# refresh-bio/kmer-db

Measured on AMD Instinct MI355X. Metric: all2all k-mer pair-comparisons/sec, higher is better.
Workload: dtype u32

## Files before the change

### kmer-db_amd/csrc/a2a_blocks.hip

```cpp
#include "device_common.h"
#include "engine_internal.h"

#include "prim.h"

#include <algorithm>
#include <chrono>
#include <cmath>
#include <cstdio>
#include <cstdlib>
#include <cstring>

enum : uint32_t {
    KCTR_CHUNKS = 0,
    KCTR_POOL_OVERFLOW,
    KCTR_PAIR_OVERFLOW,
    KCTR_NWIDE,
    KCTR_LIST_OVERFLOW,
    KCTR_RAW = 5,
    KCTR_RECORDS = 6,
    KCTR_RECORDS_HI = 7,
    KCTR_SLOW = 8,
    KCTR_WIDE_OVERFLOW = 9,
    KCTR_WIDE_RECORDS = 10,
    KCTR_ROWJOBS = 11,
// ... 815 lines not shown
                    n_direct += (uint32_t)__popcll(__ballot(mine));
                    if (!(q.dbg & 2u)) {
                    const TrConst trc = tr_const(lane);
                    const unsigned long long Rt = transpose64(mine ? F0 : 0ull, trc);
                    unsigned long long ra0, ra1;
                    {
                        const auto a = __builtin_amdgcn_permlane32_swap((uint32_t)Rt, (uint32_t)Rt, false, false);
                        const auto b = __builtin_amdgcn_permlane32_swap((uint32_t)(Rt >> 32), (uint32_t)(Rt >> 32), false, false);
                        ra0 = ((unsigned long long)b[0] << 32) | a[0];
                        ra1 = ((unsigned long long)b[1] << 32) | a[1];
                    }
                    wbuf[wave][lane] = (unsigned char)(mine ? w : 0u);
                    lds_sync();
                    const uint32_t half = lane >> 5;
                    auto spread = [&](unsigned long long word, uint32_t shift, const unsigned long long* lut) -> k2_v4i {
                        const uint32_t f = (uint32_t)(word >> shift) & 0xFFFFu;
                        k2_v4i r;
                        const unsigned long long lo = lut[f & 0xFFu], hi = lut[f >> 8];
                        r[0] = (int)(uint32_t)lo; r[1] = (int)(uint32_t)(lo >> 32); r[2] = (int)(uint32_t)hi; r[3] = (int)(uint32_t)(hi >> 32);
                        return r;
                    };
    #pragma unroll 1
                    for (uint32_t kh = 0; kh < 2; ++kh) {
                        const uint32_t shift = 32u * kh + 16u * half;
                        k2_v4i a0 = spread(ra0, shift, lut_ff), a1 = spread(ra1, shift, lut_ff);
                        const k2_v4i b0 = spread(ra0, shift, lut_01), b1 = spread(ra1, shift, lut_01);
                        const k2_v4i wv = *(const k2_v4i*)(wbuf[wave] + shift);
                        a0 &= wv; a1 &= wv;
                        c00 = __builtin_amdgcn_mfma_i32_32x32x32_i8(a0, b0, c00, 0, 0, 0);
                        c10 = __builtin_amdgcn_mfma_i32_32x32x32_i8(a1, b0, c10, 0, 0, 0);
                        c11 = __builtin_amdgcn_mfma_i32_32x32x32_i8(a1, b1, c11, 0, 0, 0);
                    }
                    lds_sync();
                    }
                    d0 = d0 && !mine;
                }
            }
            if (MODE == 0 && !q.all_wide) {
                unsigned long long pend = __ballot(d0);
                while (pend) {
                    const uint32_t X0 = bcast(w0, (uint32_t)__builtin_ctzll(pend));
                    const bool mine = d0 && w0 == X0;
                    const unsigned long long bc = __ballot(mine);
                    const Resv r = arena_reserve(A, q.pool, X0, tri32(X0) + X0, (uint32_t)__popcll(bc), lane);
                    if (mine) rec_store_diag(q.pool, resv_slot(r, (uint32_t)__popcll(bc & lt_mask)), F0, w);
                    pend &= ~bc;
                }
            } else {
                rec_emit<ROWS>(A, pv, RT, d0, w0, F0, F0, w, tri32(w0) + w0, lane, lt_mask);
            }
        };
        if (!DIRECT) first_block_records();
        {
            const bool act2 = act && F1 != 0;
            if (__ballot(act2)) {
                rec_emit<ROWS>(A, pv, RT, act2, w1, F1, F0, w, tri32(w1) + w0, lane, lt_mask);
                rec_emit<ROWS>(A, pv, RT, act2 && __popcll(F1) >= 2, w1, F1, F1, w, tri32(w1) + w1, lane, lt_mask);
            }
        }
        if (base + WAVE < end) {
            uint32_t m = dep;
#pragma unroll
            for (int s = 1; s < WAVE; s <<= 1) {
                const uint32_t o = (uint32_t)__shfl_down((int)m, s, WAVE);
                if (lane + (uint32_t)s < (uint32_t)WAVE) m = o < m ? o : m;
            }
            uint32_t later = (uint32_t)__shfl_down((int)m, 1, WAVE);
            if (lane == (uint32_t)WAVE - 1u) later = 0xFFFFFFFFu;
            if (valid && dep < later) { chain_m[dep - 1u] = make_ulonglong2(S.m0, S.m1); chain_b[dep - 1u] = S.bw; }
            lds_sync();
        }
        if (DIRECT) first_block_records();
    }
    if (DIRECT && curX != BNONE && !(q.dbg & 1u)) dflush();
    KARG(NParams) qe = kernarg_reread<NParams>();
    if (DIRECT && lane == 0 && n_direct) atomicAdd(&qe->direct_ctr[(seg % KMDB_SUBPOOLS) * 16u], n_direct);
    if (FLAT && lane == 0) { qe->slice_cnt[seg] = flat_n; if (flat_n) atomicAdd(&qe->direct_ctr[(seg % KMDB_SUBPOOLS) * 16u], flat_n); }
    if (lane == 0) qe->wide_slice_cnt[seg] = n_flagged;
    if constexpr (MODE == 0) arena_finish(A, q.pool, lane);
    if constexpr (ROWS) rowtab_finish(RT, pv, lane);
    else arena_finish_wide(A, pv, lane);
}

constexpr uint32_t K2D_SLICES = 2;
struct DParams {
    const unsigned long long* dmask;
    const uint32_t* dwx;
    const uint32_t* slice_cnt;
    uint32_t n_segs, nseg_nodes, slices;
    uint32_t* M;
    uint32_t N, bwidth;
    unsigned char* touched;
};
__global__ __launch_bounds__(256) __attribute__((amdgpu_waves_per_eu(4, 8))) void k2d_kernel(const DParams q) {
    __shared__ unsigned long long lut_ff[256], lut_01[256];
    __shared__ __attribute__((aligned(16))) unsigned char wbuf[4][64];
    {
        unsigned long long v = 0;
#pragma unroll
        for (int i = 0; i < 8; ++i) v |= ((threadIdx.x >> i) & 1u) ? 0xFFull << (8 * i) : 0ull;
        lut_ff[threadIdx.x] = v;
        lut_01[threadIdx.x] = v & 0x0101010101010101ull;
        __syncthreads();
    }
    const uint32_t lane = threadIdx.x & 63u, wave = threadIdx.x >> 6;
    const uint32_t half = lane >> 5, l31 = lane & 31u;
    const uint32_t s0 = (blockIdx.x * 4u + wave) * q.slices;
    if (s0 >= q.n_segs) return;
    const uint32_t s1 = s0 + q.slices < q.n_segs ? s0 + q.slices : q.n_segs;
    const TrConst trc = tr_const(lane);
    auto spread = [&](unsigned long long word, uint32_t shift, const unsigned long long* lut) -> k2_v4i {
        const uint32_t f = (uint32_t)(word >> shift) & 0xFFFFu;
        k2_v4i r;
        const unsigned long long lo = lut[f & 0xFFu], hi = lut[f >> 8];
        r[0] = (int)(uint32_t)lo; r[1] = (int)(uint32_t)(lo >> 32); r[2] = (int)(uint32_t)hi; r[3] = (int)(uint32_t)(hi >> 32);
        return r;
    };
    uint32_t s = s0, n = q.slice_cnt[s0], b = 0;
    auto skip_empty = [&]() { while (b >= n && s + 1u < s1) { ++s; n = q.slice_cnt[s]; b = 0; } };
    skip_empty();
    unsigned long long nm = 0; uint32_t nwx = 0;
    auto fetch = [&]() {
        nm = 0; nwx = 0;
        if (b + lane < n) { const size_t i = (size_t)s * q.nseg_nodes + b + lane; nm = q.dmask[i]; nwx = q.dwx[i]; }
    };
    if (b < n) fetch();
    unsigned long long m = 0, pend = 0;
    uint32_t wx = 0;
    auto next_step = [&]() -> bool {
        if (b >= n) return false;
        m = nm; wx = nwx;
        b += WAVE;
        skip_empty();
        if (b < n) fetch();
        pend = __ballot(m != 0ull);
        return true;
    };
    for (;;) {
        while (!pend && next_step()) {}
        if (!pend) break;
        const uint32_t X0 = bcast(wx >> 8, (uint32_t)__builtin_ctzll(pend));
        k2_v16i c00 = {}, c10 = {}, c11 = {};
        for (;;) {
            const bool mine = ((pend >> lane) & 1ull) && (wx >> 8) == X0;
            const unsigned long long bm = __ballot(mine);
            if (!bm) break;
            pend &= ~bm;
            const unsigned long long Rt = transpose64(mine ? m : 0ull, trc);
            unsigned long long ra0, ra1;
            {
                const auto a = __builtin_amdgcn_permlane32_swap((uint32_t)Rt, (uint32_t)Rt, false, false);
                const auto c = __builtin_amdgcn_permlane32_swap((uint32_t)(Rt >> 32), (uint32_t)(Rt >> 32), false, false);
                ra0 = ((unsigned long long)c[0] << 32) | a[0];
                ra1 = ((unsigned long long)c[1] << 32) | a[1];
            }
            wbuf[wave][lane] = (unsigned char)(mine ? (wx & 0xFFu) : 0u);
            lds_sync();
#pragma unroll 1
            for (uint32_t kh = 0; kh < 2; ++kh) {
                const uint32_t shift = 32u * kh + 16u * half;
                k2_v4i a0 = spread(ra0, shift, lut_ff), a1 = spread(ra1, shift, lut_ff);
                const k2_v4i b0 = spread(ra0, shift, lut_01), b1 = spread(ra1, shift, lut_01);
                const k2_v4i wv = *(const k2_v4i*)(wbuf[wave] + shift);
                a0 &= wv; a1 &= wv;
                c00 = __builtin_amdgcn_mfma_i32_32x32x32_i8(a0, b0, c00, 0, 0, 0);
                c10 = __builtin_amdgcn_mfma_i32_32x32x32_i8(a1, b0, c10, 0, 0, 0);
                c11 = __builtin_amdgcn_mfma_i32_32x32x32_i8(a1, b1, c11, 0, 0, 0);
            }
            lds_sync();
            if (pend || !next_step()) break;
        }
        const uint32_t rb = X0 * q.bwidth;
        uint32_t* const Mb = q.M + (tri64((uint64_t)rb) + rb);
        const uint32_t lim = q.N - rb;
        uint32_t h4 = 4u * half, lc = l31;
        asm volatile("" : "+v"(h4), "+v"(lc));
#pragma unroll
        for (int r = 0; r < 16; ++r) {
            const uint32_t row0 = (uint32_t)((r & 3) + 8 * (r >> 2)) + h4, row1 = row0 + 32u;
            const uint32_t o0 = rb * row0 + row0 * (row0 - 1u) / 2u + lc, o1 = rb * row1 + row1 * (row1 - 1u) / 2u + lc;
            const uint32_t v00 = (uint32_t)c00[r], v10 = (uint32_t)c10[r], v11 = (uint32_t)c11[r];
            if (v00 && lc < row0 && row0 < lim) atomicAdd(Mb + o0, v00);
            if (v10 && row1 < lim) atomicAdd(Mb + o1, v10);
            if (v11 && lc < row0 && row1 < lim) atomicAdd(Mb + o1 + 32u, v11);
        }
        if (lane == 0 && q.touched) q.touched[tri32(X0) + X0] = 1;
    }
}

constexpr uint32_t WSL_THREADS = 1024;
__global__ __launch_bounds__(WSL_THREADS) void wide_slices_kernel(const uint32_t* __restrict__ slice_cnt, uint32_t n_segs, uint32_t* __restrict__ slice_base,
                                                                   uint32_t* __restrict__ wide_base, uint32_t n_words, uint32_t* __restrict__ counters) {
    __shared__ uint32_t wtot[WSL_THREADS / WAVE];
    const uint32_t lane = threadIdx.x & 63u, wave = threadIdx.x >> 6;
    constexpr uint32_t NW = WSL_THREADS / WAVE;
    const uint32_t share = ((n_segs + NW - 1u) / NW + 63u) & ~63u;
    const uint32_t lo = wave * share < n_segs ? wave * share : n_segs;
    const uint32_t hi = n_segs - lo < share ? n_segs : lo + share;
    constexpr uint32_t U = 8;
    uint32_t sum = 0;
    for (uint32_t i0 = lo; i0 < hi; i0 += U * WAVE) {
        uint32_t v[U];
#pragma unroll
        for (uint32_t j = 0; j < U; ++j) { const uint32_t i = i0 + j * WAVE + lane; v[j] = i < hi ? slice_cnt[i] : 0u; }
#pragma unroll
        for (uint32_t j = 0; j < U; ++j) sum += v[j];
    }
#pragma unroll
    for (int d = 32; d >= 1; d >>= 1) sum += (uint32_t)__shfl_xor((int)sum, d, WAVE);
    if (lane == 0) wtot[wave] = sum;
    __syncthreads();
    uint32_t run = 0, total = 0;
    for (uint32_t k = 0; k < NW; ++k) { const uint32_t t = wtot[k]; if (k < wave) run += t; total += t; }
    for (uint32_t i0 = lo; i0 < hi; i0 += U * WAVE) {
        uint32_t v[U];
#pragma unroll
        for (uint32_t j = 0; j < U; ++j) { const uint32_t i = i0 + j * WAVE + lane; v[j] = i < hi ? slice_cnt[i] : 0u; }
#pragma unroll
        for (uint32_t j = 0; j < U; ++j) {
            const uint32_t i = i0 + j * WAVE + lane;
            const uint32_t incl = wave_incl_scan(v[j], lane);
            if (i < hi) slice_base[i] = run + incl - v[j];
            run += bcast(incl, WAVE - 1u);
        }
    }
    if (threadIdx.x == 0) { slice_base[n_segs] = total; wide_base[n_words] = total; counters[KCTR_NWIDE] = total; }
}
__global__ __launch_bounds__(256) void wide_expand_kernel(const unsigned long long* __restrict__ bits, uint32_t* __restrict__ base, const uint32_t* __restrict__ slice_base,
                                                          uint32_t words_per_slice, uint32_t slice_shift, uint32_t n_words, uint32_t* __restrict__ widx, uint32_t cap) {
    const uint32_t i = blockIdx.x * blockDim.x + threadIdx.x;
    unsigned long long b = 0;
    uint32_t o = 0;
    if (i < n_words) {
        b = bits[i];
        o = slice_base[slice_shift != 0xFFFFFFFFu ? i >> slice_shift : i / words_per_slice] + base[i];
        base[i] = o;
    }
    while (b) {
        const uint32_t k = (uint32_t)__builtin_ctzll(b);
        b &= b - 1;
        if (o < cap) widx[o] = i * 64u + k;
        ++o;
    }
}

constexpr uint32_t BLK_NONE = 0xFFFFu;
struct LSum { unsigned long long lm; uint32_t c, fb, lb; };
__device__ __forceinline__ LSum lsum_none() { return LSum{0ull, 0u, BLK_NONE, BLK_NONE}; }
__device__ __forceinline__ LSum lsum_merge(const LSum& A, const LSum& B) {
    if (B.c == 0u) return A;
    if (A.c == 0u) return B;
    const bool seam = A.lb == B.fb;
    return LSum{(B.c == 1u && seam) ? (A.lm | B.lm) : B.lm, A.c + B.c - (seam ? 1u : 0u), A.fb, B.lb};
}
__device__ __forceinline__ LSum lsum_shfl(const LSum& s, int src) {
    return LSum{shfl64(s.lm, src), (uint32_t)__shfl((int)s.c, src, WAVE), (uint32_t)__shfl((int)s.fb, src, WAVE), (uint32_t)__shfl((int)s.lb, src, WAVE)};
}
__device__ __forceinline__ LSum lsum_shfl_up(const LSum& s, int d) {
    return LSum{shfl_up64(s.lm, d), (uint32_t)__shfl_up((int)s.c, d, WAVE), (uint32_t)__shfl_up((int)s.fb, d, WAVE), (uint32_t)__shfl_up((int)s.lb, d, WAVE)};
}
__device__ __forceinline__ LSum lsum_of_fn(uint32_t fb, const ulonglong2& fm) {
    const uint32_t b0 = fb & 0xFFFFu, b1 = fb >> 16;
    if (b0 == BLK_NONE) return lsum_none();
    if (b1 == BLK_NONE) return LSum{fm.x, 1u, b0, b0};
    return LSum{fm.y, 2u, b0, b1};
}

struct L2View {
    uint32_t on, min_blocks;
    uint32_t node_cap, W;
// ... 1335 lines not shown
    const uint32_t t = blockIdx.x * blockDim.x + threadIdx.x;
    const uint64_t i0 = (uint64_t)t * q.stride + (t * 2654435761u) % q.stride;
    const uint32_t node = (uint32_t)i0;
    const bool on = i0 < q.P && q.w[node] != 0 && q.nl[node] >= 2u;
    uint32_t nblk[EST_NW], lower_first[EST_NW];
#pragma unroll
    for (int c = 0; c < EST_NW; ++c) { nblk[c] = 0; lower_first[c] = 0xFFFFFFFFu; }
    int32_t y = on ? (int32_t)node : -1;
    while (y >= 0) {
        const uint2 km = q.k0in[y];
        const uint32_t l = kmdb_k0_l(km), last = kmdb_k0_last(km);
        if (l) {
            const uint64_t pos = q.blkbase[(uint32_t)y >> 8] + q.bitrel[y];
            uint32_t sum = 0;
            if (l > 1) { BitCursor c(q.bits, pos); for (uint32_t k = 0; k + 1 < l; ++k) sum += c.next(); }
            uint32_t id = last - sum;
            uint32_t fb[EST_NW], cb[EST_NW];
#pragma unroll
            for (int c = 0; c < EST_NW; ++c) { fb[c] = __umulhi(id, q.magics[c]); cb[c] = fb[c]; nblk[c] += 1; }
            if (l > 1) {
                BitCursor c2(q.bits, pos);
                for (uint32_t k = 0; k + 1 < l; ++k) {
                    id += c2.next();
#pragma unroll
                    for (int c = 0; c < EST_NW; ++c) { const uint32_t b = __umulhi(id, q.magics[c]); nblk[c] += b != cb[c]; cb[c] = b; }
                }
            }
#pragma unroll
            for (int c = 0; c < EST_NW; ++c) { nblk[c] -= cb[c] == lower_first[c]; lower_first[c] = fb[c]; }
        }
        y = q.parent[y];
    }
    const uint32_t lane = threadIdx.x & 63u;
#pragma unroll
    for (int c = 0; c < EST_NW; ++c) {
        const unsigned long long recs = (unsigned long long)nblk[c] * (nblk[c] + 1u) / 2u;
        unsigned long long rn = on && nblk[c] >= 1u && nblk[c] <= 2u ? 1ull : 0ull;
        unsigned long long rg = on ? recs - rn : 0ull;
        unsigned long long r2 = on && nblk[c] >= q.l2_min ? recs : 0ull;
#pragma unroll
        for (int d = 32; d >= 1; d >>= 1) { rn += shfl64(rn, (int)(lane ^ (uint32_t)d)); rg += shfl64(rg, (int)(lane ^ (uint32_t)d)); r2 += shfl64(r2, (int)(lane ^ (uint32_t)d)); }
        if (lane == 0) { if (rn) atomicAdd(&q.out[c], rn); if (rg) atomicAdd(&q.out[EST_NW + c], rg); if (r2) atomicAdd(&q.out[2 * EST_NW + 1 + c], r2); }
    }
    const unsigned long long nb = __ballot(on);
    if (lane == 0 && nb) atomicAdd(&q.out[2 * EST_NW], (unsigned long long)__popcll(nb));
}

__global__ void pair_estimate_kernel(const uint2* __restrict__ k0in, const uint32_t* __restrict__ bitrel, const uint64_t* __restrict__ blkbase,
                                     const uint64_t* __restrict__ bits, uint32_t P, uint32_t stride, BlockMap bm, unsigned long long* __restrict__ out) {
    const uint32_t t = blockIdx.x * blockDim.x + threadIdx.x;
    const uint64_t i0 = (uint64_t)t * stride + (t * 2654435761u) % stride;
    unsigned long long need = 0;
    if (i0 < P) {
        const uint2 km = k0in[i0];
        const uint32_t l = kmdb_k0_l(km), last = kmdb_k0_last(km);
        if (l > 1) {
            BitCursor c(bits, blkbase[(uint32_t)i0 >> 8] + bitrel[i0]);
            uint32_t span = 0;
            for (uint32_t k = 0; k + 1 < l; ++k) span += c.next();
            const uint32_t nb = bm.blk(last) - bm.blk(last - span);
            need = nb < l - 1u ? nb : l - 1u;
        }
    }
    const uint32_t lane = threadIdx.x & 63u;
#pragma unroll
    for (int d = 32; d >= 1; d >>= 1) need += shfl64(need, (int)(lane ^ (uint32_t)d));
    if (lane == 0 && need) atomicAdd(out, need);
}

inline uint32_t wide_digit_bits(int key_bits) { return (uint32_t)(32 - key_bits - 2); }

constexpr uint32_t K1W_RUN_NODES = 256;
struct BlocksKnobs {
    uint32_t block_width = 0;
    bool dense_narrow = false;
    int k1n_mode = 2;
    int k1n_minw = 3;
    int row_mode = -1;
    bool rec_packed = true;
    bool l2 = true;
    uint32_t l2_min = L2_MIN_BLOCKS;
    uint64_t slices = 0;
    uint64_t pool_percent = 0;
    uint32_t k2d_slices = K2D_SLICES;
    bool k2d_early = true;
    uint32_t k1w_run = K1W_RUN_NODES;
    uint32_t k1w_waves = 0;
};
BlocksKnobs blocks_read_knobs() {
    BlocksKnobs k;
    auto env = [](const char* name) -> const char* { const char* e = getenv(name); return e && *e ? e : nullptr; };
    if (const char* e = env("KMDB_BLOCK_WIDTH")) { const uint32_t w = (uint32_t)strtoul(e, nullptr, 10); if (w >= 32 && w <= 64) k.block_width = w; }
    if (const char* e = env("KMDB_DENSE")) k.dense_narrow = atoi(e) >= 2;
    if (const char* e = env("KMDB_K1N_MODE")) k.k1n_mode = std::max(0, std::min(2, atoi(e)));
    if (const char* e = env("KMDB_K1N_MINW")) k.k1n_minw = atoi(e);
    if (const char* e = env("KMDB_ROW_MODE")) k.row_mode = atoi(e) != 0;
    if (const char* e = env("KMDB_REC_PACKED")) k.rec_packed = e[0] != '0';
    if (const char* e = env("KMDB_L2")) k.l2 = e[0] != '0';
    if (const char* e = env("KMDB_L2_MIN")) k.l2_min = std::max<uint32_t>(K1W_HEAVY, (uint32_t)atoi(e));
    if (const char* e = env("KMDB_SLICES")) k.slices = std::max<uint64_t>(1, strtoull(e, nullptr, 10));
    if (const char* e = env("KMDB_POOL_PERCENT")) k.pool_percent = std::max<uint64_t>(1, strtoull(e, nullptr, 10));
    if (const char* e = env("KMDB_K2D_SLICES")) k.k2d_slices = (uint32_t)std::max(1, atoi(e));
    if (const char* e = env("KMDB_K2D_EARLY")) k.k2d_early = e[0] != '0';
    if (const char* e = env("KMDB_K1W_RUN")) k.k1w_run = std::max<uint32_t>(64u, (uint32_t)atoi(e) / 64u * 64u);
    if (const char* e = env("KMDB_K1W_WAVES")) k.k1w_waves = std::max<uint32_t>(1u, (uint32_t)atoi(e));
    return k;
}
bool kmdb_verbose() { return getenv("KMDB_VERBOSE") != nullptr; }
bool kmdb_sync_debug() { return getenv("KMDB_SYNC_DEBUG") != nullptr; }
}

struct BlocksState {
    BlocksKnobs knobs;
    uint32_t NB = 0, n_states = 0;
    DevBuf<unsigned long long> p0_mask;
    DevBuf<uint32_t> p0_info;
    DevBuf<uint32_t> pair_ofs;
    DevBuf<uint16_t> pair_blk;
    DevBuf<unsigned long long> pair_mask;
    uint64_t pair_cap = 0;
    uint32_t* pair_cursor = nullptr;
    DevBuf<ulonglong2> fn_mask;
    DevBuf<uint32_t> fn_blk;
    DevBuf<unsigned long long> widebits;
    DevBuf<uint32_t> wide_base;
    DevBuf<uint32_t> wide_slice_cnt, wide_slice_base;
    DevBuf<uint32_t> widx;
    DevBuf<uint32_t> wrun_anc;
    DevBuf<uint32_t> wrun_anc_n;
    uint64_t wide_cap = 0;
    DevBuf<uint32_t> chunk_key;
    DevBuf<uint32_t> chunk_fill;
    DevBuf<uint32_t> sorted_key;
    DevBuf<uint32_t> sorted_id;
    DevBuf<void> sort_tmp;
    size_t sort_tmp_bytes = 0;
    int key_bits = 1;
    DevBuf<unsigned char> rec;
    DevBuf<uint32_t> recw;
    uint64_t pool_cap = 0;
    uint32_t* sub_cursor = nullptr;
    bool dense_narrow = false;
    int k1n_mode = 2;
    DevBuf<unsigned long long> dmask;
    DevBuf<uint32_t> dwx;
    DevBuf<uint32_t> slice_cnt;
    uint32_t* direct_ctr = nullptr;
    uint64_t last_n_direct = 0;
    DevBuf<uint32_t> wkey, swkey;
    DevBuf<WideRec> wrec, swrec;
    uint64_t wide_pool_cap = 0;
    uint32_t* wsub_cursor = nullptr;
    DevBuf<uint32_t> wide_handed;
    uint32_t* run_ctr = nullptr;
    bool row_mode = false;
    uint32_t rec_pshift = 0;
    uint32_t* ct_hist = nullptr;
    DevBuf<uint32_t> ct_offs, ct_cursor;
    DevBuf<void> ct_tmp;
    size_t ct_tmp_bytes = 0;
    DevBuf<uint32_t> rg_hist, rg_offs;
    DevBuf<uint32_t> row_ids;
    uint32_t rg_blocks = 0;
    DevBuf<void> rg_tmp;
    size_t rg_tmp_bytes = 0;
    DevBuf<uint32_t> rs_rows;
    DevBuf<uint32_t> rs_hist, rs_offs;
    uint64_t rs_entries = 0;
    DevBuf<void> rs_tmp;
    size_t rs_tmp_bytes = 0;
    uint64_t sorted_cap = 0;
    uint32_t last_n_rowjobs = 0, last_n_sorted = 0, last_n_k2jobs = 0, k1w_waves = 0, k1w_slots = 0;
    DevBuf<uint32_t> cs_hist, cs_offs;
    DevBuf<void> cs_tmp;
    size_t cs_tmp_bytes = 0;
    DevBuf<uint32_t> call_state;
    uint32_t call_state_n = 0, call_state_n_decode = 0;
    uint32_t* counters = nullptr;
    uint32_t* h_counters = nullptr;
    bool l2_on = false;
    uint32_t l2_min_blocks = 24, l2_node_cap = 0, l2_ent_cap = 0, last_l2_nodes = 0;
    DevBuf<uint32_t> l2_cursors;
    DevBuf<unsigned long long> l2_bitmap;
    DevBuf<uint32_t> l2_rank, l2_len, l2_loff;
    DevBuf<uint32_t> l2_ent_g, l2_node_w, l2_list_w;
    DevBuf<uint16_t> l2_ent_blk;
// ... 348 lines not shown
namespace {

int alloc_l2(BlocksState& b, uint32_t node_cap, uint32_t ent_cap) {
    dev_reset(b.l2_cursors, b.l2_bitmap, b.l2_rank, b.l2_len, b.l2_loff, b.l2_ent_g, b.l2_node_w, b.l2_list_w, b.l2_ent_blk, b.l2_ent_mask, b.l2_list_mask);
    b.l2_node_cap = 0; b.l2_ent_cap = 0;
    node_cap = (node_cap + 64u * L2_SUB - 1u) / (64u * L2_SUB) * (64u * L2_SUB);
    ent_cap = (ent_cap + L2_ENT_GRAB * L2_SUB - 1u) / (L2_ENT_GRAB * L2_SUB) * (L2_ENT_GRAB * L2_SUB);
    const size_t W = node_cap / 64u, NB = b.NB;
    DEV_ALLOC(b.l2_cursors, 2 * L2_SUB * 16);
    DEV_ALLOC(b.l2_bitmap, NB * W);
    DEV_ALLOC(b.l2_rank, NB * W);
    DEV_ALLOC(b.l2_len, NB);
    DEV_ALLOC(b.l2_loff, NB + 2);
    DEV_ALLOC(b.l2_ent_g, (size_t)ent_cap);
    DEV_ALLOC(b.l2_ent_blk, (size_t)ent_cap);
    DEV_ALLOC(b.l2_ent_mask, (size_t)ent_cap);
    DEV_ALLOC(b.l2_list_mask, (size_t)ent_cap);
    DEV_ALLOC(b.l2_list_w, (size_t)ent_cap);
    DEV_ALLOC(b.l2_node_w, (size_t)node_cap);
    b.l2_node_cap = node_cap; b.l2_ent_cap = ent_cap;
    return 0;
}

struct Launched { uint32_t raw = 0, rowjobs = 0, k2jobs = 0; };
inline uint32_t with_slack(uint32_t v) { return v + v / 8u + 1024u; }
int stage_done(hipStream_t s, const char* name) {
    if (!kmdb_sync_debug()) return 0;
    const hipError_t e = hipStreamSynchronize(s);
    fprintf(stderr, "[kmdb] stage %-14s %s\n", name, e == hipSuccess ? "ok" : hipGetErrorString(e));
    return e == hipSuccess ? 0 : kmdb_set_error(std::string("stage ") + name + ": " + hipGetErrorString(e));
}
void a2a_prologue(BlocksState& b, hipStream_t st, bool decode) {
    const uint32_t pool_cap = (uint32_t)b.pool_cap;
    const uint32_t n_state = decode ? b.call_state_n_decode : b.call_state_n, n_touched = decode && b.tile_touched ? b.n_states + 1u : 0u;
    hipLaunchKernelGGL(call_prologue_kernel, dim3((std::max(std::max(n_state, pool_cap), n_touched) + 255u) / 256u), dim3(256), 0, st, b.call_state.get(), n_state,
                       b.chunk_fill.get(), b.chunk_key.get(), pool_cap, b.tile_touched.get(), n_touched);
}
int a2a_decode(kmdb_db* db, BlocksState& b, hipStream_t st) {
    const uint32_t P = (uint32_t)db->P;
    K0Params q{};
    q.k0in = db->k0in; q.bitrel = db->bitrel; q.blkbase = db->blkbase; q.bits = db->bits; q.perm = nullptr; q.P = P; q.short_ids = db->short_max_ids;
    q.bm = BlockMap{db->width, (uint32_t)((1ull << 32) / db->width) + 1u};
    q.p0_mask = b.p0_mask; q.p0_info = b.p0_info; q.pair_ofs = b.pair_ofs; q.pair_blk = b.pair_blk; q.pair_mask = b.pair_mask;
    uint32_t nreg = 1;
    while (nreg < KMDB_PAIR_REGIONS && (uint64_t)nreg * 16384 < P) nreg <<= 1;
    q.pair_cursor = b.pair_cursor; q.n_regions = nreg; q.region_cap = (uint32_t)(b.pair_cap * 3 / 4 / nreg);
    q.spill_cap = (uint32_t)(b.pair_cap - (uint64_t)q.region_cap * nreg); q.counters = b.counters;
    hipLaunchKernelGGL((k0_decode_kernel<false>), dim3((P + 255) / 256), dim3(256), 0, st, q);
    if (db->n_long) {
        q.perm = db->long_nodes; q.P = db->n_long;
        hipLaunchKernelGGL((k0_decode_kernel<true>), dim3((db->n_long + 255) / 256), dim3(256), 0, st, q);
    }
    HIP_TRY(hipGetLastError());
    return 0;
}
int a2a_narrow_emit(kmdb_db* db, BlocksState& b, uint32_t* M, uint32_t emit_lo, uint32_t emit_hi, hipStream_t st) {
    NParams q{};
    q.nl = db->nl; q.parent = db->parent; q.w = db->w; q.dflag = db->dflag; q.seg_anc = db->nseg_anc; q.seg_anc_n = db->nseg_anc_n;
    q.p0_mask = b.p0_mask; q.p0_info = b.p0_info; q.pair_ofs = b.pair_ofs; q.pair_blk = b.pair_blk; q.pair_mask = b.pair_mask;
    q.fn_mask = b.fn_mask; q.fn_blk = b.fn_blk; q.widebits = b.widebits; q.wide_base = b.wide_base; q.wide_slice_cnt = b.wide_slice_cnt;
    q.P = (uint32_t)db->P; q.nseg_nodes = db->nseg_nodes; q.n_segs = db->n_nsegs; q.chain_cap = db->chain_cap;
    q.emit_lo = emit_lo; q.emit_hi = emit_hi; q.tbits = b.dense_narrow ? 0u : arena_table_bits(b.NB); q.n_keys = b.NB;
    q.all_wide = b.dense_narrow ? 1u : 0u;
    q.pool = pool_view(b, b.dense_narrow);
    const size_t wave_lds = k1n_wave_bytes(q.chain_cap, q.tbits, q.n_keys, b.row_mode ? b.NB : 0u);
    const uint32_t waves = (uint32_t)std::max<size_t>(1, std::min<size_t>(K1N_WAVES, (144u << 10) / wave_lds));
    const size_t lds = wave_lds * waves;
    q.M = M; q.N = (uint32_t)db->N; q.bwidth = db->width; q.touched = b.tile_touched; q.direct_ctr = b.direct_ctr;
    q.dmask = b.dmask; q.dwx = b.dwx; q.slice_cnt = b.slice_cnt;
    const K1nPick pick = k1n_pick(b.k1n_mode, b.knobs.k1n_minw, b.row_mode);
    HIP_TRY(hipFuncSetAttribute((const void*)pick.fn, hipFuncAttributeMaxDynamicSharedMemorySize, (int)lds));
    const dim3 grid((q.n_segs + waves - 1) / waves), block(WAVE * waves);
    if (!b.have_counts && kmdb_verbose())
        fprintf(stderr, "[kmdb] narrow kernel: %u slices, %zu B of LDS per wave, %u per workgroup, instantiation %s\n", q.n_segs, wave_lds, waves, pick.name);
    hipLaunchKernelGGL(pick.fn, grid, block, lds, st, q);
    HIP_TRY(hipGetLastError());
    return 0;
}
int a2a_slice_apply(kmdb_db* db, BlocksState& b, uint32_t* M, hipStream_t st, hipStream_t s2) {
    HIP_TRY(hipEventRecord(db->ev_side[0], st));
    HIP_TRY(hipStreamWaitEvent(s2, db->ev_side[0], 0));
    DParams d{};
    d.dmask = b.dmask; d.dwx = b.dwx; d.slice_cnt = b.slice_cnt; d.n_segs = db->n_nsegs; d.nseg_nodes = db->nseg_nodes;
    const uint32_t sl = b.knobs.k2d_slices;
    d.slices = sl; d.M = M; d.N = (uint32_t)db->N; d.bwidth = db->width; d.touched = b.tile_touched;
    const uint32_t waves = (db->n_nsegs + sl - 1u) / sl;
    if (waves) hipLaunchKernelGGL(k2d_kernel, dim3((waves + 3u) / 4u), dim3(256), 0, s2, d);
    HIP_TRY(hipGetLastError());
    HIP_TRY(hipEventRecord(db->ev_side[1], s2));
    (void)stage_done(s2, "slice apply");
    return 0;
}
int a2a_group_and_apply_chunks(kmdb_db* db, BlocksState& b, uint32_t* M, hipStream_t cs, hipStream_t s2) {
    const uint32_t pool_cap = (uint32_t)b.pool_cap;
    hipLaunchKernelGGL(ct_hist_kernel, dim3((pool_cap + CT_THREADS - 1) / CT_THREADS), dim3(CT_THREADS), 0, cs, b.chunk_key, pool_cap, b.n_states, b.ct_hist);
    size_t tb = b.ct_tmp_bytes;
    HIP_TRY(prim::exclusive_sum(b.ct_tmp, tb, b.ct_hist, b.ct_offs.get(), (int)(b.n_states + 1), cs));
    HIP_TRY(hipMemcpyAsync(b.ct_cursor, b.ct_offs, ((size_t)b.n_states + 1) * 4, hipMemcpyDeviceToDevice, cs));
    hipLaunchKernelGGL(ct_scatter_kernel, dim3((pool_cap + CT_THREADS - 1) / CT_THREADS), dim3(CT_THREADS), 0, cs, b.chunk_key, pool_cap, b.n_states, b.ct_cursor, b.sorted_key, b.sorted_id);
    hipLaunchKernelGGL(ct_count_kernel, dim3(1), dim3(1), 0, cs, b.ct_offs, b.n_states, b.counters);
    if (cs != s2) { HIP_TRY(hipEventRecord(db->ev_side[0], cs)); HIP_TRY(hipStreamWaitEvent(s2, db->ev_side[0], 0)); }
    {
        rocprim::transform_iterator<uint32_t*, U32toU64, unsigned long long> it(b.chunk_fill, U32toU64());
        HIP_TRY(prim::sum(b.sort_tmp, b.sort_tmp_bytes, it, (unsigned long long*)(b.counters + KCTR_RECORDS), (int)pool_cap, s2));
    }
    const uint32_t win = b.n_states <= CS_MAX_KEYS ? 16u : 32u;
    uint32_t grid = (pool_cap + win - 1) / win;
    if (b.have_counts) grid = std::min(grid, (b.last_n_chunks + win - 1) / win);
    if (grid)
        hipLaunchKernelGGL(k2_apply_kernel, dim3(grid), dim3(256), 0, s2, b.rec, b.recw, b.sorted_key, b.sorted_id, b.chunk_fill, b.n_states,
                           b.ct_offs + b.n_states, M, (uint32_t)db->N, db->width, win, b.tile_touched);
    HIP_TRY(hipGetLastError());
    HIP_TRY(hipEventRecord(db->ev_side[1], s2));
    (void)stage_done(s2, "chunk apply");
    return 0;
}
int a2a_wide_list(kmdb_db* db, BlocksState& b, hipStream_t st, uint32_t* n_wide_out) {
    const uint32_t n_words = ((uint32_t)db->P + 63) / 64;
    hipLaunchKernelGGL(wide_slices_kernel, dim3(1), dim3(WSL_THREADS), 0, st, b.wide_slice_cnt.get(), db->n_nsegs, b.wide_slice_base.get(), b.wide_base.get(), n_words,
                       b.counters);
    uint32_t n_wide;
    if (b.have_counts && b.wide_cap >= b.last_n_wide) n_wide = b.last_n_wide;
    else {
        HIP_TRY(hipMemcpyAsync(b.h_counters, b.counters + KCTR_NWIDE, 4, hipMemcpyDeviceToHost, st));
        HIP_TRY(hipStreamSynchronize(st));
        n_wide = b.h_counters[0];
        if (n_wide > b.wide_cap) {
            dev_reset(b.widx, b.wrun_anc, b.wrun_anc_n);
            b.wide_cap = 0;
            DEV_ALLOC(b.widx, (size_t)n_wide);
            DEV_ALLOC(b.wrun_anc, ((size_t)n_wide / 64 + 1) * db->chain_cap);
            DEV_ALLOC(b.wrun_anc_n, (size_t)n_wide / 64 + 1);
            b.wide_cap = n_wide;
        }
    }
    if (!b.widx) { DEV_ALLOC(b.widx, 1); b.wide_cap = std::max<uint64_t>(b.wide_cap, 1); }
    const uint32_t wps = db->nseg_nodes / 64u;
    hipLaunchKernelGGL(wide_expand_kernel, dim3((n_words + 255) / 256), dim3(256), 0, st, b.widebits.get(), b.wide_base.get(),
                       b.wide_slice_base.get(), wps, (wps & (wps - 1u)) ? 0xFFFFFFFFu : (uint32_t)__builtin_ctz(wps), n_words, b.widx.get(), (uint32_t)b.wide_cap);
    *n_wide_out = n_wide;
    return 0;
}
int a2a_wide_emit(kmdb_db* db, BlocksState& b, uint32_t* M, uint32_t emit_lo, uint32_t emit_hi, uint32_t n_wide, hipStream_t st) {
    WParams q{};
    q.widx = b.widx; q.n_wide = n_wide; q.nl = db->nl; q.parent = db->parent; q.w = db->w; q.widebits = b.widebits;
    q.dflag = db->dflag; q.wide_base = b.wide_base;
    q.p0_mask = b.p0_mask; q.p0_info = b.p0_info; q.pair_ofs = b.pair_ofs; q.pair_blk = b.pair_blk; q.pair_mask = b.pair_mask;
    q.fn_mask = b.fn_mask; q.fn_blk = b.fn_blk; q.emit_lo = emit_lo; q.emit_hi = emit_hi; q.pool = pool_view(b, true);
    if (b.l2_on && !b.l2_bitmap) {
        const bool tiny = b.knobs.pool_percent != 0;
        if (alloc_l2(b, tiny ? 1u : std::max<uint32_t>(64u * L2_SUB * 4u, n_wide / 16u), tiny ? 1u : std::max<uint32_t>(L2_ENT_GRAB * L2_SUB * 4u, n_wide / 16u * 48u))) return 1;
    }
    q.l2 = L2View{};
    if (b.l2_on) {
        q.l2.on = 1u; q.l2.min_blocks = b.l2_min_blocks; q.l2.node_cap = b.l2_node_cap; q.l2.W = b.l2_node_cap / 64u; q.l2.ent_cap = b.l2_ent_cap;
        q.l2.cursors = b.l2_cursors; q.l2.bitmap = b.l2_bitmap; q.l2.ent_g = b.l2_ent_g; q.l2.ent_blk = b.l2_ent_blk; q.l2.ent_mask = b.l2_ent_mask;
        q.l2.node_w = b.l2_node_w;
        HIP_TRY(hipMemsetAsync(b.l2_cursors, 0, 2 * L2_SUB * 16 * 4, st));
        HIP_TRY(hipMemsetAsync(b.l2_bitmap, 0, (size_t)b.NB * q.l2.W * 8, st));
        HIP_TRY(hipMemsetAsync(b.l2_ent_blk, 0xFF, (size_t)b.l2_ent_cap * 2, st));
    }
    q.run_nodes = b.knobs.k1w_run;
    q.n_runs = (n_wide + q.run_nodes - 1) / q.run_nodes;
    hipLaunchKernelGGL(wrun_anc_kernel, dim3((q.n_runs + 63) / 64), dim3(64), 0, st, b.widx, n_wide, q.run_nodes, db->parent, db->dflag, db->chain_cap,
                       b.wrun_anc, b.wrun_anc_n);
    q.seg_anc = b.wrun_anc; q.seg_anc_n = b.wrun_anc_n;
    q.chain_cap = db->chain_cap; q.e_cap = (b.NB + 2u + 3u) & ~3u; q.arena_cap = std::max<uint32_t>(K1W_ARENA_MIN, (b.NB + 2u + 63u) & ~63u);
// ... 123 lines not shown
            want = 0;
        } else if ((want << CH_SHIFT) >= pool_slot_limit(b)) {
            if (b.n_slices >= (1u << 16)) {
                db->fallback_reason = "more block records than a pool can index in a 65536th of the patterns (" + std::to_string(b.n_states) + " streams, " + std::to_string(b.pool_cap) + " chunks were not enough)";
                return 0;
            }
            b.n_slices *= 2;
            if (verbose) fprintf(stderr, "[kmdb] record pool at its limit: %u slices of the pattern stream per call\n", b.n_slices);
            return 0;
        }
        if (want) {
            if (verbose) fprintf(stderr, "[kmdb] record pool too small (%llu chunks): %llu\n", (unsigned long long)b.pool_cap, (unsigned long long)want);
            if (alloc_record_pool(b, db->stream, want)) return 1;
        }
    }
    return 0;
}
int a2a_settle(kmdb_db* db, BlocksState& b, hipStream_t st, const Launched& L, bool* retry) {
    const bool row_mode = b.row_mode;
    HIP_TRY(hipMemcpyAsync(b.h_counters, b.counters, KCTR_COUNT * 4, hipMemcpyDeviceToHost, st));
    HIP_TRY(hipStreamSynchronize(st));
    const uint32_t* c = b.h_counters;
    if (c[KCTR_LIST_OVERFLOW] || c[KCTR_SLOW]) {
        db->fallback_reason = "internal: the wide-node kernel lost a list (chain miss " + std::to_string(c[KCTR_SLOW]) + ", arena overflow " + std::to_string(c[KCTR_LIST_OVERFLOW]) + ")";
        return 0;
    }
    if (c[KCTR_L2_OVERFLOW]) {
        if (kmdb_verbose()) fprintf(stderr, "[kmdb] second level out of node indices or entries (%u / %u): doubling\n", b.l2_node_cap, b.l2_ent_cap);
        if (alloc_l2(b, b.l2_node_cap * 2u, b.l2_ent_cap * 2u)) return 1;
        b.have_counts = false; *retry = true;
        return 0;
    }
    if (c[KCTR_PAIR_OVERFLOW] || c[KCTR_POOL_OVERFLOW] || c[KCTR_WIDE_OVERFLOW]) {
        if (a2a_enlarge_pools(db, b, c)) return 1;
        if (db->fallback_reason.empty()) { b.have_counts = false; *retry = true; }
        return 0;
    }
    if (b.have_counts && (c[KCTR_NWIDE] != b.last_n_wide || c[KCTR_CHUNKS] != b.last_n_chunks ||
                            (row_mode ? (c[KCTR_ROWJOBS] > L.rowjobs || c[KCTR_WIDE_RECORDS] != b.last_n_sorted || c[KCTR_K2JOBS] > L.k2jobs)
                                      : (c[KCTR_RAW] > L.raw || c[KCTR_K2JOBS] > L.k2jobs)))) {
        if (kmdb_verbose())
            fprintf(stderr, "[kmdb] a launch was sized too small (wide nodes %u / %u, chunks %u / %u, row jobs %u / %u, sorted %u / %u, apply jobs %u / %u, raw %u / %u): the call is repeated\n",
                    c[KCTR_NWIDE], b.last_n_wide, c[KCTR_CHUNKS], b.last_n_chunks, c[KCTR_ROWJOBS], L.rowjobs, c[KCTR_WIDE_RECORDS], b.last_n_sorted, c[KCTR_K2JOBS],
                    L.k2jobs, c[KCTR_RAW], L.raw);
        b.have_counts = false; *retry = true;
        return 0;
    }
    if ((uint64_t)c[KCTR_POOL_USED] * 100 > b.pool_cap * 85) {
        if (kmdb_verbose()) fprintf(stderr, "[kmdb] record pool %u of %llu chunks in use: enlarged by a quarter\n", c[KCTR_POOL_USED], (unsigned long long)b.pool_cap);
        const uint64_t want = b.pool_cap + b.pool_cap / 4;
        if (((want + (uint64_t)KMDB_SUBPOOLS * ARENA_GRAB) << CH_SHIFT) < pool_slot_limit(b) && alloc_record_pool(b, db->stream, want)) return 1;
    }
    if (!row_mode && (uint64_t)c[KCTR_RAW] * 100 > b.wide_pool_cap * 85) {
        if (kmdb_verbose()) fprintf(stderr, "[kmdb] wide record pool %u of %llu chunks in use: enlarged by a quarter\n", c[KCTR_RAW], (unsigned long long)b.wide_pool_cap);
        const uint64_t want = b.wide_pool_cap + b.wide_pool_cap / 4;
        if (((want + (uint64_t)KMDB_SUBPOOLS * WIDE_GRAB) << WCH_SHIFT) < pool_slot_limit(b) && alloc_wide_pool(b, db->stream, want)) return 1;
    }
    if (!b.have_counts && kmdb_verbose())
        fprintf(stderr, "[kmdb] record pool: %u of %llu chunks in use (busiest sub-pool x sub-pools); wide pool / sorted arrays: %llu slots\n", c[KCTR_POOL_USED],
                (unsigned long long)b.pool_cap, (unsigned long long)b.sorted_cap);
    b.last_n_wide = c[KCTR_NWIDE]; b.last_n_chunks = c[KCTR_CHUNKS]; b.last_n_raw = c[KCTR_RAW];
    b.last_n_rowjobs = c[KCTR_ROWJOBS]; b.last_n_sorted = c[KCTR_WIDE_RECORDS]; b.last_l2_nodes = c[KCTR_L2_NODES]; b.last_n_k2jobs = c[KCTR_K2JOBS];
    if (b.l2_on && !b.have_counts && kmdb_verbose())
        fprintf(stderr, "[kmdb] second level: %u nodes with %u blocks or more joined per tile (indices for %u, entries for %u)\n", c[KCTR_L2_NODES], b.l2_min_blocks,
                b.l2_node_cap, b.l2_ent_cap);
    b.last_records = ((uint64_t)c[KCTR_RECORDS] | ((uint64_t)c[KCTR_RECORDS_HI] << 32)) + (row_mode ? 0u : c[KCTR_WIDE_RECORDS]);
    b.last_n_direct = c[KCTR_DIRECT];
    return 0;
}
int blocks_attempt(kmdb_db* db, uint32_t* M, uint32_t emit_lo, uint32_t emit_hi, bool decode, hipStream_t st, bool* retry) {
    BlocksState& b = *db->blocks;
    hipStream_t s2 = db->stream2;
    *retry = false;
    Launched L;
    if (b.have_counts) L.raw = (uint32_t)std::min<uint64_t>(with_slack(b.last_n_raw), b.row_mode ? 0xFFFFFFFFull : b.wide_pool_cap);
    a2a_prologue(b, st, decode);
    if (stage_done(st, "init")) return 1;
    if (decode && a2a_decode(db, b, st)) return 1;
    if (stage_done(st, "decode")) return 1;
    HIP_TRY(hipEventRecord(db->ev_k[0], st));
    if (a2a_narrow_emit(db, b, M, emit_lo, emit_hi, st)) return 1;
    if (stage_done(st, "narrow emit")) return 1;
    HIP_TRY(hipEventRecord(db->ev_k[1], st));
    if (b.k1n_mode == 2 && b.knobs.k2d_early && a2a_slice_apply(db, b, M, st, s2)) return 1;
    if (!b.row_mode) {
        if (!b.dense_narrow) {
            HIP_TRY(hipEventRecord(db->ev_side[0], st));
            HIP_TRY(hipStreamWaitEvent(s2, db->ev_side[0], 0));
            if (a2a_group_and_apply_chunks(db, b, M, s2, s2)) return 1;
        } else HIP_TRY(hipEventRecord(db->ev_side[1], s2));
    }
    uint32_t n_wide = 0;
    if (a2a_wide_list(db, b, st, &n_wide)) return 1;
    if (b.k1n_mode == 2 && !b.knobs.k2d_early && a2a_slice_apply(db, b, M, st, s2)) return 1;
    if (n_wide && a2a_wide_emit(db, b, M, emit_lo, emit_hi, n_wide, st)) return 1;
    HIP_TRY(hipGetLastError());
    if (stage_done(st, "wide emit")) return 1;
    HIP_TRY(hipEventRecord(db->ev_k[2], st));
    if (b.row_mode ? a2a_sort_apply_rows(db, b, M, st, s2, L) : a2a_sort_apply_flat(db, b, M, st, L)) return 1;
    if (stage_done(st, b.row_mode ? "row sort+apply" : "sorted apply")) return 1;
    HIP_TRY(hipStreamWaitEvent(st, db->ev_side[1], 0));
    hipLaunchKernelGGL(pool_used_kernel, dim3(1), dim3(64), 0, st, b.sub_cursor, b.direct_ctr, b.counters);
    HIP_TRY(hipEventRecord(db->ev_k[3], st));
    return a2a_settle(db, b, st, L, retry);
}

}

static void blocks_join_side_streams(kmdb_db* db) {
    if (db->stream2) (void)hipStreamSynchronize(db->stream2);
}

int kmdb_blocks_run(kmdb_db* db, uint32_t* M, uint32_t emit_lo, uint32_t emit_hi, hipStream_t st) {
    BlocksState& b = *db->blocks;
    const uint64_t cells = db->N * (db->N - 1) / 2;
    for (int round = 0; round < 64; ++round) {
        const uint32_t S = std::max<uint32_t>(1u, b.n_slices);
        bool again = false;
        uint64_t records = 0, direct = 0;
        if (b.slice_counts.size() != S) b.slice_counts.assign(S, BlocksState::SliceCounts{});
        bool decoded = false;
        db->last_call_sized = false;
        for (uint32_t k = 0; k < S && !again; ++k) {
            const uint32_t lo = emit_lo + (uint32_t)((uint64_t)(emit_hi - emit_lo) * k / S), hi = emit_lo + (uint32_t)((uint64_t)(emit_hi - emit_lo) * (k + 1) / S);
            if (lo == hi) continue;
            BlocksState::SliceCounts& sc = b.slice_counts[k];
            b.have_counts = sc.valid && sc.lo == lo && sc.hi == hi;
            if (b.have_counts) { b.last_n_wide = sc.n_wide; b.last_n_chunks = sc.n_chunks; b.last_n_raw = sc.n_raw; b.last_n_rowjobs = sc.n_rowjobs; b.last_n_sorted = sc.n_sorted; b.last_n_k2jobs = sc.n_k2jobs; }
            if (!b.have_counts) db->last_call_sized = true;
            bool retry = false;
            if (blocks_attempt(db, M, lo, hi, !decoded, st, &retry)) { blocks_join_side_streams(db); return 1; }
            decoded = true;
            if (!db->fallback_reason.empty()) return 0;
            if (retry) { again = true; for (auto& c : b.slice_counts) c.valid = false; }
            else {
                sc = BlocksState::SliceCounts{true, lo, hi, b.last_n_wide, b.last_n_chunks, b.last_n_raw, b.last_n_rowjobs, b.last_n_sorted, b.last_n_k2jobs};
                records += b.last_records;
                direct += b.last_n_direct;
            }
        }
        if (!again) { b.last_records = records; b.last_n_direct = direct; b.have_counts = true; return 0; }
        HIP_TRY(hipMemsetAsync(M, 0, cells * 4, st));
    }
    return kmdb_set_error("kmdb_blocks_run: the record pools did not converge");
}

kmdb_blocks_counts kmdb_blocks_last_counts(const kmdb_db* db) {
    const BlocksState& b = *db->blocks;
    return kmdb_blocks_counts{b.last_records, b.last_n_direct, b.last_n_wide, b.last_n_chunks, b.l2_on ? b.last_l2_nodes : 0u};
}
const unsigned char* kmdb_blocks_tile_touched(const kmdb_db* db) { return db->blocks ? db->blocks->tile_touched.get() : nullptr; }
```

Baseline: 20820 billion.

## Accumulate k2d dense-tile results in LDS, adapt slices, and launch after wide emit

Each k2d block now claims one output tile in shared memory through an atomicCAS tag. Waves whose tile matches the claimed one accumulate their MFMA results with LDS atomics instead of global atomics. At the end the block flushes the tile once to M. The per-wave slice count now defaults to a value that grows with segment count, and the slice-apply launch moves by default to after the wide emit. This is meant to cut global atomic traffic and kernel count, at the cost of about 8KB extra LDS per block (lower occupancy), a tile zeroing pass, and changed overlap with the other streams.

```diff
diff --git a/kmer-db_amd/csrc/a2a_blocks.hip b/kmer-db_amd/csrc/a2a_blocks.hip
--- a/kmer-db_amd/csrc/a2a_blocks.hip
+++ b/kmer-db_amd/csrc/a2a_blocks.hip
@@ -921,7 +921,15 @@
     else arena_finish_wide(A, pv, lane);
 }
 
-constexpr uint32_t K2D_SLICES = 2;
+constexpr uint32_t K2D_SLICES_MIN = 2, K2D_SLICES_MAX = 32, K2D_WAVES = 1500;
+constexpr uint32_t K2D_TILE_WORDS = 64 * 63 / 2;
+constexpr uint32_t K2D_NO_TILE = 0xFFFFFFFFu;
+inline uint32_t k2d_default_slices(uint32_t n_segs) {
+    uint32_t s = K2D_SLICES_MIN;
+    while (s < K2D_SLICES_MAX && n_segs / (2u * s) >= K2D_WAVES) s *= 2u;
+    return s;
+}
+inline uint32_t k2d_clamp_slices(uint32_t s, uint32_t nseg_nodes) { return std::max(1u, std::min(s, (1u << 24) / std::max(nseg_nodes, 1u))); }
 struct DParams {
     const unsigned long long* dmask;
     const uint32_t* dwx;
@@ -934,19 +942,23 @@
 __global__ __launch_bounds__(256) __attribute__((amdgpu_waves_per_eu(4, 8))) void k2d_kernel(const DParams q) {
     __shared__ unsigned long long lut_ff[256], lut_01[256];
     __shared__ __attribute__((aligned(16))) unsigned char wbuf[4][64];
+    __shared__ uint32_t tile[K2D_TILE_WORDS];
+    __shared__ uint32_t tile_tag;
     {
         unsigned long long v = 0;
 #pragma unroll
         for (int i = 0; i < 8; ++i) v |= ((threadIdx.x >> i) & 1u) ? 0xFFull << (8 * i) : 0ull;
         lut_ff[threadIdx.x] = v;
         lut_01[threadIdx.x] = v & 0x0101010101010101ull;
+        for (uint32_t i = threadIdx.x; i < K2D_TILE_WORDS; i += 256u) tile[i] = 0u;
+        if (threadIdx.x == 0) tile_tag = K2D_NO_TILE;
         __syncthreads();
     }
     const uint32_t lane = threadIdx.x & 63u, wave = threadIdx.x >> 6;
     const uint32_t half = lane >> 5, l31 = lane & 31u;
     const uint32_t s0 = (blockIdx.x * 4u + wave) * q.slices;
-    if (s0 >= q.n_segs) return;
-    const uint32_t s1 = s0 + q.slices < q.n_segs ? s0 + q.slices : q.n_segs;
+    const bool any = s0 < q.n_segs;
+    const uint32_t s1 = !any ? s0 : s0 + q.slices < q.n_segs ? s0 + q.slices : q.n_segs;
     const TrConst trc = tr_const(lane);
     auto spread = [&](unsigned long long word, uint32_t shift, const unsigned long long* lut) -> k2_v4i {
         const uint32_t f = (uint32_t)(word >> shift) & 0xFFFFu;
@@ -955,7 +967,7 @@
         r[0] = (int)(uint32_t)lo; r[1] = (int)(uint32_t)(lo >> 32); r[2] = (int)(uint32_t)hi; r[3] = (int)(uint32_t)(hi >> 32);
         return r;
     };
-    uint32_t s = s0, n = q.slice_cnt[s0], b = 0;
+    uint32_t s = s0, n = any ? q.slice_cnt[s0] : 0u, b = 0;
     auto skip_empty = [&]() { while (b >= n && s + 1u < s1) { ++s; n = q.slice_cnt[s]; b = 0; } };
     skip_empty();
     unsigned long long nm = 0; uint32_t nwx = 0;
@@ -1009,11 +1021,26 @@
             lds_sync();
             if (pend || !next_step()) break;
         }
+        uint32_t h4 = 4u * half, lc = l31;
+        asm volatile("" : "+v"(h4), "+v"(lc));
+        uint32_t tag = 0;
+        if (lane == 0) tag = atomicCAS(&tile_tag, K2D_NO_TILE, X0);
+        tag = bcast(tag, 0);
+        if (tag == K2D_NO_TILE || tag == X0) {
+#pragma unroll
+            for (int r = 0; r < 16; ++r) {
+                const uint32_t row0 = (uint32_t)((r & 3) + 8 * (r >> 2)) + h4, row1 = row0 + 32u;
+                const uint32_t o0 = row0 * (row0 - 1u) / 2u + lc, o1 = row1 * (row1 - 1u) / 2u + lc;
+                const uint32_t v00 = (uint32_t)c00[r], v10 = (uint32_t)c10[r], v11 = (uint32_t)c11[r];
+                if (v00 && lc < row0) atomicAdd(tile + o0, v00);
+                if (v10) atomicAdd(tile + o1, v10);
+                if (v11 && lc < row0) atomicAdd(tile + o1 + 32u, v11);
+            }
+            continue;
+        }
         const uint32_t rb = X0 * q.bwidth;
         uint32_t* const Mb = q.M + (tri64((uint64_t)rb) + rb);
         const uint32_t lim = q.N - rb;
-        uint32_t h4 = 4u * half, lc = l31;
-        asm volatile("" : "+v"(h4), "+v"(lc));
 #pragma unroll
         for (int r = 0; r < 16; ++r) {
             const uint32_t row0 = (uint32_t)((r & 3) + 8 * (r >> 2)) + h4, row1 = row0 + 32u;
@@ -1025,6 +1052,20 @@
         }
         if (lane == 0 && q.touched) q.touched[tri32(X0) + X0] = 1;
     }
+    __syncthreads();
+    const uint32_t XT = tile_tag;
+    if (XT == K2D_NO_TILE) return;
+    const uint32_t rb = XT * q.bwidth;
+    uint32_t* const Mb = q.M + (tri64((uint64_t)rb) + rb);
+    const uint32_t lim = q.N - rb < 64u ? q.N - rb : 64u;
+    for (uint32_t r = 1u + (threadIdx.x >> 5); r < lim; r += 8u) {
+        const uint32_t t = r * (r - 1u) / 2u;
+        for (uint32_t c = l31; c < r; c += 32u) {
+            const uint32_t v = tile[t + c];
+            if (v) atomicAdd(Mb + (rb * r + t + c), v);
+        }
+    }
+    if (threadIdx.x == 0 && q.touched) q.touched[tri32(XT) + XT] = 1;
 }
 
 constexpr uint32_t WSL_THREADS = 1024;
@@ -2526,8 +2567,8 @@
     uint32_t l2_min = L2_MIN_BLOCKS;
     uint64_t slices = 0;
     uint64_t pool_percent = 0;
-    uint32_t k2d_slices = K2D_SLICES;
-    bool k2d_early = true;
+    uint32_t k2d_slices = 0;
+    int k2d_early = 2;
     uint32_t k1w_run = K1W_RUN_NODES;
     uint32_t k1w_waves = 0;
 };
@@ -2545,7 +2586,7 @@
     if (const char* e = env("KMDB_SLICES")) k.slices = std::max<uint64_t>(1, strtoull(e, nullptr, 10));
     if (const char* e = env("KMDB_POOL_PERCENT")) k.pool_percent = std::max<uint64_t>(1, strtoull(e, nullptr, 10));
     if (const char* e = env("KMDB_K2D_SLICES")) k.k2d_slices = (uint32_t)std::max(1, atoi(e));
-    if (const char* e = env("KMDB_K2D_EARLY")) k.k2d_early = e[0] != '0';
+    if (const char* e = env("KMDB_K2D_EARLY")) k.k2d_early = e[0] == '0' ? 0 : e[0] == '1' ? 1 : 2;
     if (const char* e = env("KMDB_K1W_RUN")) k.k1w_run = std::max<uint32_t>(64u, (uint32_t)atoi(e) / 64u * 64u);
     if (const char* e = env("KMDB_K1W_WAVES")) k.k1w_waves = std::max<uint32_t>(1u, (uint32_t)atoi(e));
     return k;
@@ -3060,7 +3101,7 @@
     HIP_TRY(hipStreamWaitEvent(s2, db->ev_side[0], 0));
     DParams d{};
     d.dmask = b.dmask; d.dwx = b.dwx; d.slice_cnt = b.slice_cnt; d.n_segs = db->n_nsegs; d.nseg_nodes = db->nseg_nodes;
-    const uint32_t sl = b.knobs.k2d_slices;
+    const uint32_t sl = k2d_clamp_slices(b.knobs.k2d_slices ? b.knobs.k2d_slices : k2d_default_slices(db->n_nsegs), db->nseg_nodes);
     d.slices = sl; d.M = M; d.N = (uint32_t)db->N; d.bwidth = db->width; d.touched = b.tile_touched;
     const uint32_t waves = (db->n_nsegs + sl - 1u) / sl;
     if (waves) hipLaunchKernelGGL(k2d_kernel, dim3((waves + 3u) / 4u), dim3(256), 0, s2, d);
@@ -3350,7 +3391,7 @@
     if (a2a_narrow_emit(db, b, M, emit_lo, emit_hi, st)) return 1;
     if (stage_done(st, "narrow emit")) return 1;
     HIP_TRY(hipEventRecord(db->ev_k[1], st));
-    if (b.k1n_mode == 2 && b.knobs.k2d_early && a2a_slice_apply(db, b, M, st, s2)) return 1;
+    if (b.k1n_mode == 2 && b.knobs.k2d_early == 1 && a2a_slice_apply(db, b, M, st, s2)) return 1;
     if (!b.row_mode) {
         if (!b.dense_narrow) {
             HIP_TRY(hipEventRecord(db->ev_side[0], st));
@@ -3360,8 +3401,9 @@
     }
     uint32_t n_wide = 0;
     if (a2a_wide_list(db, b, st, &n_wide)) return 1;
-    if (b.k1n_mode == 2 && !b.knobs.k2d_early && a2a_slice_apply(db, b, M, st, s2)) return 1;
+    if (b.k1n_mode == 2 && b.knobs.k2d_early == 0 && a2a_slice_apply(db, b, M, st, s2)) return 1;
     if (n_wide && a2a_wide_emit(db, b, M, emit_lo, emit_hi, n_wide, st)) return 1;
+    if (b.k1n_mode == 2 && b.knobs.k2d_early == 2 && a2a_slice_apply(db, b, M, st, s2)) return 1;
     HIP_TRY(hipGetLastError());
     if (stage_done(st, "wide emit")) return 1;
     HIP_TRY(hipEventRecord(db->ev_k[2], st));
```

After: 21220 billion, median of 6. No clear change (+1.9%).
